# AutonomousVehicleLaboratory/vision_semantic_segmentation

Hardware: AMD Instinct MI355X
Metric: fused frames/sec/GPU (1920x1080 + 120k pts) + max|dlog-odds| vs ref (higher is better)
Workload: dtype f16 hi+lo split, MX-FP4 correction passes, fp32 accumulate

## Files before the change

### vision_semantic_segmentation_amd/csrc/experiments/seg_gemm_mx_pp.inc

```

template <int IO>
__global__ void __launch_bounds__(512) k_gemm_mx_pp(MxArgs q, int mtiles) {
    typedef f16 H;
    typedef typename Half16<H>::v8 v8;
    typedef int v8i __attribute__((ext_vector_type(8)));
    constexpr int MI = 8, BM = 256, BN = 256;
    constexpr int A_BYTES = BM * 128, W_BYTES = BN * 128;
    constexpr int W_REGION = 2 * A_BYTES, S_REGION = W_REGION + 2 * W_BYTES, S_BYTES = 4096;
    extern __shared__ __attribute__((aligned(16))) char lds[];
    const GemmArgs& p = q.g;

    const int tid = threadIdx.x, lane = tid & 63;
    const int wave = __builtin_amdgcn_readfirstlane(tid >> 6);
    const int wm = wave >> 2, wn = wave & 3;
    const int nwg = gridDim.x;
    int vb;
    {
        const int bid = blockIdx.x, xcd = bid & 7, local = bid >> 3, qq = nwg >> 3, r = nwg & 7;
        vb = (xcd < r ? xcd * (qq + 1) : r * (qq + 1) + (xcd - r) * qq) + local;
    }
    const int ntiles = p.ntiles, nmx = q.nmx;
    const int total = mtiles * ntiles;
    const int nmb = p.K / 256;
    const int nsub = 4 + nmx;
    const unsigned lds_base = lds_addr(lds);

    auto lane_now = [&]() __attribute__((always_inline)) {
        unsigned l;
        asm volatile("v_mbcnt_lo_u32_b32 %0, -1, 0\n\tv_mbcnt_hi_u32_b32 %0, -1, %0" : "=v"(l));
        return l;
    };
    int pt = vb, pmb = 0, pj = 0, issued = 0, pmbl = 0;
    long long cur_rowb16 = 0, cur_rowbq = 0, cur_asrows = 0;
    const char *cur_a16 = nullptr, *cur_aq = nullptr, *cur_as = nullptr, *cur_w16 = nullptr, *cur_wq = nullptr, *cur_ws = nullptr;
// ... 190 lines not shown
#pragma unroll
            for (int n = 0; n < 2; ++n) asm volatile("" : "+v"(acc[4 * I + m][2 * J + n]));
        __builtin_amdgcn_sched_barrier(0);
    };
    auto close = [&]() __attribute__((always_inline)) {
        asm volatile("s_barrier" ::: "memory");
        __builtin_amdgcn_sched_barrier(0);
    };
    typedef std::integral_constant<int, 0> F16;
    typedef std::integral_constant<int, 1> FP4;
    typedef std::integral_constant<int, 0> Q0;
    typedef std::integral_constant<int, 1> Q1;
    typedef std::integral_constant<int, 2> Q2;
    typedef std::integral_constant<int, 3> Q3;

    asm volatile("s_waitcnt vmcnt(0)\n\ts_barrier" ::: "memory");
    if (wm == 1) asm volatile("s_barrier" ::: "memory");
    __builtin_amdgcn_sched_barrier(0);
    for (int t = vb; t < total; t += nwg) {
        const int nt = t % ntiles, mt = t / ntiles;
        for (int mb = 0; mb < nmb; ++mb) {
            const bool last_mb = mb + 1 == nmb;
            for (int j = 0; j < 4; ++j) {
                quadrant(F16(), Q0()); close(); quadrant(F16(), Q1()); close(); quadrant(F16(), Q2()); close(); quadrant(F16(), Q3()); close();
                ++g;
            }
            for (int u = 0; u < nmx; ++u) {
                quadrant(FP4(), Q0()); close(); quadrant(FP4(), Q1()); close(); quadrant(FP4(), Q2()); close(); quadrant(FP4(), Q3());
                if (!(last_mb && u + 1 == nmx)) close();
                ++g;
            }
        }
        if (wm == 0) close();
        mx_epilogue<IO, MI>(q, acc, nt, mt, wm, wn, fr, kq);
        if (t + nwg < total) init_acc(t + nwg);
        if (wm == 1) close();
    }
    if (wm == 0) asm volatile("s_barrier" ::: "memory");
}
```

### vision_semantic_segmentation_amd/csrc/seg_gemm.hip

```cpp
#include <cstdlib>
#include <cstring>
#include <type_traits>

#include "seg_types.h"

namespace avl {
namespace {

struct GemmArgs {
    const void* A;
    const void* W;
    const float* bias;
    const void* R;
    void* C;
    int lda, ldr, ldc;
    int M, N, K;
    int relu, out_f32;
    int ntiles;
    int nsub;
    long long a_lo_delta;
    const void* R_lo;
    void* C_lo;
};

template <int NSUB> __device__ __forceinline__ bool sub_needs_a(int j) { return NSUB == 1 || j == 0 || (NSUB == 3 && j == 2); }

__device__ __forceinline__ void glds16(const void* g, void* l) {
    __builtin_amdgcn_global_load_lds((const __attribute__((address_space(1))) void*)g,
                                     (__attribute__((address_space(3))) void*)l, 16, 0, 0);
}

template <typename T, int WM, int WN>
__global__ void __launch_bounds__(WM* WN * 64) k_gemm(GemmArgs p) {
    constexpr int NW = WM * WN, BM = WM * 64, BN = WN * 64;
    constexpr int A_BYTES = BM * 128, W_BYTES = BN * 128, BUF = A_BYTES + W_BYTES;
// ... 422 lines not shown
    a.ntiles = (a.N + BN - 1) / BN;
    const int mtiles = (M + BM - 1) / BM;
    const int total = mtiles * a.ntiles;
    const int grid = total < 256 ? total : 256;
#ifdef AVL_EXPERIMENTS
    const int probe = AVL_EXP_INT("AVL_GEMM_PROBE", 0);
    if (probe >= 1 && probe <= 3 && NSUB == 1 && IO == 0) {
#define AVL_PROBE_LAUNCH(P)                                                                                                                     \
    do {                                                                                                                                        \
        (void)hipFuncSetAttribute(reinterpret_cast<const void*>(&k_gemm_ring<H, WM, WN, MI, STAGES, P>), hipFuncAttributeMaxDynamicSharedMemorySize, LDS); \
        hipLaunchKernelGGL((k_gemm_ring<H, WM, WN, MI, STAGES, P>), dim3(grid), dim3(WM * WN * 64), LDS, s, a, mtiles);                         \
    } while (0)
        if (probe == 1) AVL_PROBE_LAUNCH(1);
        else if (probe == 2) AVL_PROBE_LAUNCH(2);
        else AVL_PROBE_LAUNCH(3);
#undef AVL_PROBE_LAUNCH
    } else
#endif
        hipLaunchKernelGGL((k_gemm_ring<H, WM, WN, MI, STAGES, 0, NSUB, IO, AST>), dim3(grid), dim3(WM * WN * 64), LDS, s, a, mtiles);
    AVL_LAUNCH_CHECK();
    return AVL_OK;
}

template <typename T, int WM, int WN>
int launch_cfg(const GemmArgs& a, int mtiles, hipStream_t s) {
    constexpr int LDS = 2 * (WM * 64 + WN * 64) * 128;
    AVL_HIP_CHECK(hipFuncSetAttribute(reinterpret_cast<const void*>(&k_gemm<T, WM, WN>),
                                      hipFuncAttributeMaxDynamicSharedMemorySize, LDS));
    hipLaunchKernelGGL((k_gemm<T, WM, WN>), dim3(mtiles * a.ntiles), dim3(WM * WN * 64), LDS, s, a);
    AVL_LAUNCH_CHECK();
    return AVL_OK;
}

struct MxArgs {
    GemmArgs g;
    const char* Aq[2];
    const char* As[2];
    const char* Wq[2];
    const char* Ws[2];
    int ldaq;
    long long a_srows, w_srows;
    char* Cq[2];
    char* Cs[2];
    int ldcq;
    long long c_srows;
    int nmx;
    const char* Rq;
    const char* Rs;
    int ldrq;
    long long r_srows;
    int nmb1;
    const void* A2;
    int lda2, ldaq2;
    const char* Aq2[2];
    const char* As2[2];
    long long a_srows2;
    int stagger;
    unsigned long long* dbg;
    int same_tile;
};

__device__ __forceinline__ unsigned quantize_fp4_block(const float (&v)[16], unsigned (&q)[2]) {
    float amax = 0.f;
#pragma unroll
    for (int i = 0; i < 16; ++i) amax = fmaxf(amax, fabsf(v[i]));
    {
        const unsigned ab = __float_as_uint(amax);
        const auto r16 = __builtin_amdgcn_permlane16_swap(ab, ab, false, false);
        amax = __uint_as_float(max(r16[0], r16[1]));
    }
    const unsigned sbyte = mx_fp4_scale_byte(amax);
    const float scale = __uint_as_float(sbyte << 23);
    q[0] = q[1] = 0u;
#define AVL_FP4_PAIR(i)                                                                                  \
    q[0] = __builtin_amdgcn_cvt_scalef32_pk_fp4_f32(q[0], v[2 * (i)], v[2 * (i) + 1], scale, (i));        \
    q[1] = __builtin_amdgcn_cvt_scalef32_pk_fp4_f32(q[1], v[8 + 2 * (i)], v[8 + 2 * (i) + 1], scale, (i))
    AVL_FP4_PAIR(0); AVL_FP4_PAIR(1); AVL_FP4_PAIR(2); AVL_FP4_PAIR(3);
#undef AVL_FP4_PAIR
    return sbyte;
}

template <int IO, int MI>
__device__ __forceinline__ void mx_epilogue(const MxArgs& q, f32x4 (&acc)[MI][4], int nt, int mt, int wm, int wn, int fr, int kq) {
    typedef f16 H;
    typedef typename Half16<H>::v8 v8;
    constexpr int BM = 2 * MI * 16, BN = 256;
    const GemmArgs& p = q.g;
    const int nbase = nt * BN + wn * 64 + kq * 16;
    const bool ncol_ok = nbase + 16 <= p.N;
    const bool rsplit = p.R_lo != nullptr, csplit = p.C_lo != nullptr;
    const unsigned m0 = (unsigned)(mt * BM + wm * (MI * 16) + fr);
    const unsigned sc_r = (unsigned)(nbase >> 8) * (unsigned)q.r_srows * 8u + (unsigned)((nbase >> 5) & 7);
    const unsigned sc_c = (unsigned)(nbase >> 8) * (unsigned)q.c_srows * 8u + (unsigned)((nbase >> 5) & 7);
    v8 nr0 = {}, nr1 = {};
    uint2 npk = make_uint2(0u, 0u);
    unsigned nsb = 127u;
    auto load_res = [&](int mi) {
        const unsigned m = m0 + mi * 16;
        if (p.R && (int)m < p.M && ncol_ok) {
            const H* rp = static_cast<const H*>(p.R) + (m * (unsigned)p.ldr + (unsigned)nbase);
            nr0 = *reinterpret_cast<const v8*>(rp);
            nr1 = *reinterpret_cast<const v8*>(rp + 8);
            if (q.Rq) {
                npk = *reinterpret_cast<const uint2*>(q.Rq + (m * (unsigned)q.ldrq + (unsigned)(nbase / 2)));
                nsb = (unsigned char)q.Rs[sc_r + m * 8u];
            }
        }
    };
    load_res(0);
#pragma unroll
    for (int mi = 0; mi < MI; ++mi) {
        const unsigned m = m0 + mi * 16;
        const bool live = (int)m < p.M && ncol_ok;
        const v8 r0 = nr0, r1 = nr1;
        const uint2 pk = npk;
        const unsigned sb = nsb;
        if (mi + 1 < MI) load_res(mi + 1);
        float v[16];
#pragma unroll
        for (int nj = 0; nj < 4; ++nj)
#pragma unroll
            for (int r = 0; r < 4; ++r) v[nj * 4 + r] = acc[mi][nj][r];
        if (p.R && live) {
            float rl[16];
#pragma unroll
            for (int i = 0; i < 16; ++i) rl[i] = 0.f;
            if (rsplit) {
                const H* rlp = static_cast<const H*>(p.R_lo) + (m * (unsigned)p.ldr + (unsigned)nbase);
                const v8 l0 = *reinterpret_cast<const v8*>(rlp), l1 = *reinterpret_cast<const v8*>(rlp + 8);
#pragma unroll
                for (int i = 0; i < 8; ++i) { rl[i] = (float)l0[i]; rl[8 + i] = (float)l1[i]; }
            } else if (q.Rq) {
                typedef float v2f __attribute__((ext_vector_type(2)));
                const float sc = __uint_as_float(sb << 23);
#define AVL_FP4_DEC(w, sel, o) { const v2f d = __builtin_amdgcn_cvt_scalef32_pk_f32_fp4(w, sc, sel); rl[o] = d.x; rl[o + 1] = d.y; }
                AVL_FP4_DEC(pk.x, 0, 0) AVL_FP4_DEC(pk.x, 1, 2) AVL_FP4_DEC(pk.x, 2, 4) AVL_FP4_DEC(pk.x, 3, 6)
                AVL_FP4_DEC(pk.y, 0, 8) AVL_FP4_DEC(pk.y, 1, 10) AVL_FP4_DEC(pk.y, 2, 12) AVL_FP4_DEC(pk.y, 3, 14)
#undef AVL_FP4_DEC
            }
#pragma unroll
            for (int i = 0; i < 8; ++i) { v[i] += (float)r0[i] + rl[i]; v[8 + i] += (float)r1[i] + rl[8 + i]; }
        }
        if (p.relu) {
#pragma unroll
            for (int i = 0; i < 16; ++i) v[i] = fmaxf(v[i], 0.f);
        }
        v8 h0, h1;
#pragma unroll
        for (int i = 0; i < 8; ++i) { h0[i] = (H)v[i]; h1[i] = (H)v[8 + i]; }
        float hi[16], lo[16];
#pragma unroll
        for (int i = 0; i < 8; ++i) {
            hi[i] = (float)h0[i];
            hi[8 + i] = (float)h1[i];
            lo[i] = v[i] - hi[i];
            lo[8 + i] = v[8 + i] - hi[8 + i];
        }
        const unsigned coff = m * (unsigned)p.ldc + (unsigned)nbase;
        if (live) {
            H* cp = static_cast<H*>(p.C) + coff;
            *reinterpret_cast<v8*>(cp) = h0;
            *reinterpret_cast<v8*>(cp + 8) = h1;
        }
        if (csplit) {
            v8 l0, l1;
#pragma unroll
            for (int i = 0; i < 8; ++i) { l0[i] = (H)lo[i]; l1[i] = (H)lo[8 + i]; }
            if (live) {
                H* cl = static_cast<H*>(p.C_lo) + coff;
                *reinterpret_cast<v8*>(cl) = l0;
                *reinterpret_cast<v8*>(cl + 8) = l1;
            }
#pragma unroll
            for (int i = 0; i < 8; ++i) { lo[i] = (float)l0[i]; lo[8 + i] = (float)l1[i]; }
        }
        if constexpr (IO != 0) {
#pragma unroll
            for (int pl = 0; pl < 2; ++pl) {
                if (q.Cq[pl] == nullptr) continue;
                unsigned pq[2];
                const unsigned sq = quantize_fp4_block(pl == 0 ? hi : lo, pq);
                if (live) {
                    *reinterpret_cast<uint2*>(q.Cq[pl] + (m * (unsigned)q.ldcq + (unsigned)(nbase / 2))) = make_uint2(pq[0], pq[1]);
                    if ((kq & 1) == 0) q.Cs[pl][sc_c + m * 8u] = (char)sq;
                }
            }
        }
    }
}

template <int IO, int MI>
__global__ void __launch_bounds__(512) k_gemm_ring_mx(MxArgs q, int mtiles) {
    typedef f16 H;
    typedef typename Half16<H>::v8 v8;
    typedef int v8i __attribute__((ext_vector_type(8)));
    constexpr int WM = 2, WN = 4, STAGES = 2;
    constexpr int NW = WM * WN, BM = WM * MI * 16, BN = WN * 64;
    constexpr int A_BYTES = BM * 128, W_BYTES = BN * 128;
    constexpr int W_REGION = STAGES * A_BYTES, S_REGION = W_REGION + STAGES * W_BYTES;
    constexpr int S_BYTES = 4096;
    constexpr int A_INSTR = BM / 8 / NW, W_INSTR = BN / 8 / NW;
    extern __shared__ __attribute__((aligned(16))) char lds[];
    const GemmArgs& p = q.g;

    const int tid = threadIdx.x, lane = tid & 63;
    const int wave = __builtin_amdgcn_readfirstlane(tid >> 6);
    const int wm = wave / WN, wn = wave % WN;
    const int nwg = gridDim.x;
    int vb;
    {
        const int bid = blockIdx.x, xcd = bid & 7, local = bid >> 3, qq = nwg >> 3, r = nwg & 7;
        vb = (xcd < r ? xcd * (qq + 1) : r * (qq + 1) + (xcd - r) * qq) + local;
    }
    const int total = mtiles * p.ntiles;
    const int nmb = p.K / 256;
    const int nsub = 4 + q.nmx;
    const unsigned lds_base = lds_addr(lds);

    const int srow = lane >> 3, schunk = lane & 7;
    const unsigned ct = (unsigned)((schunk ^ srow) << 4);
    const unsigned a_lane16 = (unsigned)srow * (unsigned)(p.lda * 2) + ct, a_laneq = (unsigned)srow * (unsigned)q.ldaq + ct;
    const unsigned a_lane16_2 = (unsigned)srow * (unsigned)(q.lda2 * 2) + ct, a_laneq_2 = (unsigned)srow * (unsigned)q.ldaq2 + ct;
    unsigned w_off16[W_INSTR], w_offq[W_INSTR];
#pragma unroll
// ... 105 lines not shown
                for (int kk = 0; kk < 2; ++kk) {
                    if (kk == late && pt < total) issue();
                    int4 wf[4];
                    int ws[4];
#pragma unroll
                    for (int nj = 0; nj < 4; ++nj) {
                        wf[nj] = *reinterpret_cast<const int4*>(wbase + w_off[nj] + (((kk * 4 + kq) ^ w_key[nj]) << 4));
                        {
                            const uint2 w8 = *reinterpret_cast<const uint2*>(sbase + 2048 + (wn * 4 + (fr >> 2)) * 128 + ((fr & 3) * 4 + kq) * 8);
                            ws[nj] = (int)(((nj < 2 ? w8.x : w8.y) >> (8 * ((nj & 1) * 2 + kk))) & 0xffu);
                        }
                    }
                    const int achunk = ((kk * 4 + kq) ^ a_key) << 4;
                    int4 af = *reinterpret_cast<const int4*>(abase + achunk);
                    unsigned asw = *reinterpret_cast<const unsigned*>(sbase + a_row0 * 8 + kk * 4);
#pragma unroll
                    for (int mi = 0; mi < MI; ++mi) {
                        const int4 cur = af;
                        const int as = (int)((asw >> (8 * kq)) & 0xffu);
                        if (mi + 1 < MI) {
                            af = *reinterpret_cast<const int4*>(abase + (mi + 1) * 2048 + achunk);
                            asw = *reinterpret_cast<const unsigned*>(sbase + (a_row0 + (mi + 1) * 16) * 8 + kk * 4);
                        }
                        const v8i xa = {cur.x, cur.y, cur.z, cur.w, 0, 0, 0, 0};
#pragma unroll
                        for (int nj = 0; nj < 4; ++nj) {
                            const v8i wa = {wf[nj].x, wf[nj].y, wf[nj].z, wf[nj].w, 0, 0, 0, 0};
                            acc[mi][nj] = __builtin_amdgcn_mfma_scale_f32_16x16x128_f8f6f4(wa, xa, acc[mi][nj], 4, 4, 0, ws[nj], 0, as);
                        }
                    }
                }
            }
        }
        mx_epilogue<IO, MI>(q, acc, nt, mt, wm, wn, fr, kq);
        if (t + nwg < total) init_acc(t + nwg);
    }
}

template <int IO, int MI, int LATE, int PROBE = 0, int SPREAD = 0>
__global__ void __launch_bounds__(512) k_gemm_mx_pipe(MxArgs q, int mtiles) {
    typedef f16 H;
    typedef typename Half16<H>::v8 v8;
    typedef int v8i __attribute__((ext_vector_type(8)));
    constexpr int WM = 2, WN = 4, STAGES = 2;
    constexpr int NW = WM * WN, BM = WM * MI * 16, BN = WN * 64;
    constexpr int A_BYTES = BM * 128, W_BYTES = BN * 128;
    constexpr int W_REGION = STAGES * A_BYTES, S_REGION = W_REGION + STAGES * W_BYTES;
    constexpr int S_BYTES = 4096;
    constexpr int A_INSTR = BM / 8 / NW, W_INSTR = BN / 8 / NW;
    constexpr int NS = 2 * MI, D = 3, EV = NS - D;
    constexpr int EW = (MI == 8 && SPREAD != 5) ? 5 : EV;
    constexpr bool SPR = SPREAD == 1 || SPREAD == 2, PIN = SPREAD != 0;
    constexpr bool ONE = SPREAD == 5;
    constexpr bool MID = SPREAD == 4;
    extern __shared__ __attribute__((aligned(16))) char lds[];
    const GemmArgs& p = q.g;

    const int tid = threadIdx.x, lane = tid & 63;
    const int wave = __builtin_amdgcn_readfirstlane(tid >> 6);
    const int wm = wave / WN, wn = wave % WN;
    const int nwg = gridDim.x;
    int vb;
    {
        const int bid = blockIdx.x, xcd = bid & 7, local = bid >> 3, qq = nwg >> 3, r = nwg & 7;
        vb = (xcd < r ? xcd * (qq + 1) : r * (qq + 1) + (xcd - r) * qq) + local;
    }
    const int ntiles = p.ntiles, nmx = q.nmx;
    const int total = mtiles * ntiles;
    const int nmb = p.K / 256;
    const int nsub = 4 + nmx;
    const unsigned lds_base = lds_addr(lds);

// ... 92 lines not shown
    if (pt < total) { issue_w(); issue_a(); }
    if (pt < total) { issue_w(); issue_a(); }

    const int fr = lane & 15, kq = lane >> 4;
    const int a_row0 = wm * (MI * 16) + fr;
    const int wrow0 = wn * 64 + (fr >> 2) * 16 + (fr & 3);
    const int wkey_r = ((wrow0 >> 1) & 1) | (((wrow0 >> 4) & 3) << 1);
    const unsigned a_v0 = (unsigned)(a_row0 * 128 + ((kq ^ (a_row0 & 7)) << 4));
    const unsigned w_v0 = (unsigned)(W_REGION + wrow0 * 128 + ((kq ^ wkey_r) << 4));
    const unsigned sa_v = (unsigned)(S_REGION + a_row0 * 8 + kq);
    const unsigned sw_v = (unsigned)(S_REGION + 2048 + (wn * 4 + (fr >> 2)) * 128 + ((fr & 3) * 4 + kq) * 8);

    f32x4 acc[MI][4];
    auto init_acc = [&](int t) {
        const int nb = (t % ntiles) * BN + wn * 64 + kq * 16;
#pragma unroll
        for (int nj = 0; nj < 4; ++nj) {
            const float4 b = *reinterpret_cast<const float4*>(p.bias + nb + 4 * nj);
#pragma unroll
            for (int mi = 0; mi < MI; ++mi) acc[mi][nj] = f32x4{b.x, b.y, b.z, b.w};
        }
    };
    if (vb < total) init_acc(vb);

    int4 Af[NS], Wf[2][4];
    unsigned As[NS];
    uint2 Wsc = make_uint2(0u, 0u), Wsn = make_uint2(0u, 0u);
    auto rdA = [&](const char* slot, int kk, int mi) { return *reinterpret_cast<const int4*>(slot + (a_v0 ^ (unsigned)(kk * 64)) + mi * 2048); };
    auto rdW = [&](const char* slot, int kk, int nj) { return *reinterpret_cast<const int4*>(slot + (w_v0 ^ (unsigned)(kk * 64)) + nj * 512); };
    auto rdAs = [&](const char* slot, int kk, int mi) { return (unsigned)*reinterpret_cast<const unsigned char*>(slot + sa_v + mi * 128 + kk * 4); };
    auto rdWs = [&](const char* slot) { return *reinterpret_cast<const uint2*>(slot + sw_v); };

    int g = 0;
    unsigned long long tsum[8] = {0, 0, 0, 0, 0, 0, 0, 0}, tlast = 0;
    auto stamp = [&]() __attribute__((always_inline)) {
        unsigned long long t;
        asm volatile("s_memtime %0\n\ts_waitcnt lgkmcnt(0)" : "=s"(t)::"memory");
        return t;
    };
    bool w_sent = false;
    auto step = [&](auto kind_c, auto s_c, const bool next_q) __attribute__((always_inline)) {
        constexpr int KIND = decltype(kind_c)::value, S = decltype(s_c)::value;
        constexpr int kk = S / MI, mi = S % MI;
        const char* ab = lds + (g & 1) * A_BYTES;
        const char* wb = lds + (g & 1) * W_BYTES;
        const char* sb = lds + (g & 1) * S_BYTES;
        const char* abn = lds + ((g + 1) & 1) * A_BYTES;
        const char* wbn = lds + ((g + 1) & 1) * W_BYTES;
        const char* sbn = lds + ((g + 1) & 1) * S_BYTES;
        auto readA = [&](int t) {
            Af[t] = rdA(ab, t / MI, t % MI);
            if (KIND == 1) As[t] = rdAs(sb, t / MI, t % MI);
        };
        auto readAn = [&](int t) {
            Af[t] = rdA(abn, t / MI, t % MI);
            As[t] = rdAs(sbn, t / MI, t % MI);
        };
        if (PROBE == 3 && S == 0) { const unsigned long long t = stamp(); if (tlast) tsum[0] += t - tlast; tlast = t; tsum[5] += 1; }
        if (EW != EV && S == EW) {
            if (!SPR && !MID && LATE == 0 && !early && g > 0 && PROBE != 1 && pt < total) {
                unsigned long long t1 = 0;
                if (PROBE == 3) t1 = stamp();
                issue_a();
                if (PROBE == 3) tsum[4] += stamp() - t1;
            }
            unsigned long long t0 = 0;
            if (PROBE == 3) t0 = stamp();
// ... 100 lines not shown
            for (int nj = 0; nj < 4; ++nj) asm volatile("" : "+v"(acc[mi][nj]));
        }
        __builtin_amdgcn_sched_barrier(0);
    };
    auto substep = [&](auto kind_c, const bool next_q) __attribute__((always_inline)) {
#define AVL_STEP(N) step(kind_c, std::integral_constant<int, N>(), next_q)
        AVL_STEP(0); AVL_STEP(1); AVL_STEP(2); AVL_STEP(3); AVL_STEP(4); AVL_STEP(5); AVL_STEP(6); AVL_STEP(7);
        if constexpr (NS == 16) { AVL_STEP(8); AVL_STEP(9); AVL_STEP(10); AVL_STEP(11); AVL_STEP(12); AVL_STEP(13); AVL_STEP(14); AVL_STEP(15); }
#undef AVL_STEP
        Wsc = Wsn;
        ++g;
    };
    typedef std::integral_constant<int, 0> F16;
    typedef std::integral_constant<int, 1> FP4;

    asm volatile("s_waitcnt vmcnt(0)" ::: "memory");
    __builtin_amdgcn_s_barrier();
    for (int t = vb; t < total; t += nwg) {
        const int nt = t % ntiles, mt = t / ntiles;
        {
            const char* ab = lds + (g & 1) * A_BYTES;
            const char* wb = lds + (g & 1) * W_BYTES;
#pragma unroll
            for (int nj = 0; nj < 4; ++nj) Wf[0][nj] = rdW(wb, 0, nj);
#pragma unroll
            for (int s = 0; s < D; ++s) Af[s] = rdA(ab, 0, s);
        }
        for (int mb = 0; mb < nmb; ++mb) {
            for (int j = 0; j < 4; ++j) substep(F16(), j == 3);
            for (int u = 0; u < nmx; ++u) substep(FP4(), u + 1 < nmx);
        }
        unsigned long long te0 = 0;
        if (PROBE == 3) te0 = stamp();
        mx_epilogue<IO, MI>(q, acc, nt, mt, wm, wn, fr, kq);
        if (t + nwg < total) init_acc(t + nwg);
        if (PROBE == 3) { tsum[6] += stamp() - te0; tsum[7] += 1; tlast = 0; }
    }
    if (PROBE == 3 && q.dbg && lane == 0) {
#pragma unroll
        for (int i = 0; i < 8; ++i) q.dbg[((size_t)blockIdx.x * 8 + wave) * 8 + i] = tsum[i];
    }
}

#ifdef AVL_EXPERIMENTS
#include "experiments/seg_gemm_mx_pp.inc"
#endif

template <int IO, int MI>
int launch_ring_mx_t(const MxArgs& a0, hipStream_t s) {
    constexpr int BM = 2 * MI * 16, LDS = 2 * (BM + 256) * 128 + 2 * 4096;
    MxArgs a = a0;
    a.stagger = AVL_EXP_INT("AVL_MX_STAGGER", 1);
    a.same_tile = 0;
    a.g.ntiles = a.g.N / 256;
    const int mtiles = (a.g.M + BM - 1) / BM;
    const int total = mtiles * a.g.ntiles;
    int grid = total < 256 ? total : 256;
#ifdef AVL_EXPERIMENTS
    { const int gl = AVL_EXP_INT("AVL_MX_GRID", 0); if (gl > 0 && gl < grid) grid = gl; }
#endif
#ifdef AVL_EXPERIMENTS
    if (MI == 8) {
        const int pp = AVL_EXP_INT("AVL_MX_PP", 0);
        if (pp == 1 || (pp == 2 && a.g.K >= 1024)) {
            AVL_HIP_CHECK(hipFuncSetAttribute(reinterpret_cast<const void*>(&k_gemm_mx_pp<IO>), hipFuncAttributeMaxDynamicSharedMemorySize, LDS));
            hipLaunchKernelGGL((k_gemm_mx_pp<IO>), dim3(grid), dim3(512), LDS, s, a, mtiles);
            AVL_LAUNCH_CHECK();
            return AVL_OK;
        }
    }
#endif
    const int pipe_env = AVL_EXP_INT("AVL_MX_PIPE", -1);
    const bool pipe = pipe_env >= 0 ? pipe_env != 0 : a.g.K >= 1024;
    if (pipe) {
        constexpr int L0 = MI == 8 ? 0 : 1;
#define AVL_PIPE_LAUNCH(...)                                                                                                                   \
    do {                                                                                                                                       \
        AVL_HIP_CHECK(hipFuncSetAttribute(reinterpret_cast<const void*>(&k_gemm_mx_pipe<__VA_ARGS__>), hipFuncAttributeMaxDynamicSharedMemorySize, LDS)); \
        hipLaunchKernelGGL((k_gemm_mx_pipe<__VA_ARGS__>), dim3(grid), dim3(512), LDS, s, a, mtiles);                                           \
    } while (0)
#ifdef AVL_EXPERIMENTS
        constexpr int L1 = 2;
        const int late_env = AVL_EXP_INT("AVL_MX_LATE", -1);
        const int probe = AVL_EXP_INT("AVL_MX_PROBE", 0);
        if (MI == 8 && probe == 1) AVL_PIPE_LAUNCH(IO, 8, 0, 1);
        else if (MI == 8 && probe == 2) AVL_PIPE_LAUNCH(IO, 8, 0, 2);
        else if (MI == 8 && probe == 4) AVL_PIPE_LAUNCH(IO, 8, 0, 4);
        else if (MI == 8 && probe == 5) AVL_PIPE_LAUNCH(IO, 8, 0, 5);
        else if (MI == 8 && probe == 6) AVL_PIPE_LAUNCH(IO, 8, 0, 6);
        else if (MI == 8 && probe == 3) {
            hipStreamCaptureStatus cap = hipStreamCaptureStatusNone;
            AVL_HIP_CHECK(hipStreamIsCapturing(s, &cap));
            AVL_REQUIRE(cap == hipStreamCaptureStatusNone, "AVL_MX_PROBE=3 synchronises the stream: not while it is being captured (MODEL.HIP_GRAPH = False)");
            static unsigned long long* dbg = nullptr;
            if (!dbg) AVL_HIP_CHECK(hipHostMalloc(reinterpret_cast<void**>(&dbg), 256 * 8 * 8 * sizeof(unsigned long long), 0));
            memset(dbg, 0, 256 * 8 * 8 * sizeof(unsigned long long));
            a.dbg = dbg;
            a.same_tile = AVL_EXP_INT("AVL_MX_SAMETILE", 0);
            AVL_PIPE_LAUNCH(IO, 8, 0, 3);
            AVL_HIP_CHECK(hipStreamSynchronize(s));
            double sum[2][8] = {};
            for (int b = 0; b < grid; ++b)
                for (int w = 0; w < 8; ++w)
                    for (int i = 0; i < 8; ++i) sum[w >= 4][i] += (double)dbg[(b * 8 + w) * 8 + i];
            for (int e = 0; e < 2; ++e) {
                const double n = sum[e][5] > 0 ? sum[e][5] : 1;
                fprintf(stderr, "[mx probe] M %d N %d K %d nmx %d %s waves: cycles per sub-step %.0f | EW wait+barrier %.0f | W burst %.0f | EV wait+barrier %.0f | A burst %.0f | epilogue %.0f (x %.1f per wave)\n",
                        a.g.M, a.g.N, a.g.K, a.nmx, e ? "early (4-7)" : "late (0-3)", sum[e][0] / n, sum[e][1] / n, sum[e][2] / n, sum[e][3] / n, sum[e][4] / n,
                        sum[e][7] > 0 ? sum[e][6] / sum[e][7] : 0., sum[e][7] / (4.0 * grid));
            }
        }
        else if (late_env == L1) AVL_PIPE_LAUNCH(IO, MI, L1);
        else if (MI == 8 && AVL_EXP_INT("AVL_MX_SPREAD", 0) == 1) AVL_PIPE_LAUNCH(IO, 8, 0, 0, 1);
        else if (MI == 8 && AVL_EXP_INT("AVL_MX_SPREAD", 0) == 2) AVL_PIPE_LAUNCH(IO, 8, 0, 0, 2);
        else if (MI == 8 && AVL_EXP_INT("AVL_MX_SPREAD", 0) == 3) AVL_PIPE_LAUNCH(IO, 8, 0, 0, 3);
        else if (MI == 8 && AVL_EXP_INT("AVL_MX_SPREAD", 0) == 4) AVL_PIPE_LAUNCH(IO, 8, 0, 0, 4);
        else if (MI == 8 && AVL_EXP_INT("AVL_MX_SPREAD", 0) == 5) AVL_PIPE_LAUNCH(IO, 8, 0, 0, 5);
        else
#endif
            AVL_PIPE_LAUNCH(IO, MI, L0);
#undef AVL_PIPE_LAUNCH
    } else {
        AVL_HIP_CHECK(hipFuncSetAttribute(reinterpret_cast<const void*>(&k_gemm_ring_mx<IO, MI>), hipFuncAttributeMaxDynamicSharedMemorySize, LDS));
        hipLaunchKernelGGL((k_gemm_ring_mx<IO, MI>), dim3(grid), dim3(512), LDS, s, a, mtiles);
    }
    AVL_LAUNCH_CHECK();
    return AVL_OK;
}

int launch_ring_mx(const MxArgs& a, bool quantize_out, hipStream_t s) {
    const int force = AVL_EXP_INT("AVL_MX_TILE", 0);
    const long long t256 = (long long)((a.g.M + 255) / 256) * (a.g.N / 256);
    const bool small = force ? force == 128 : (t256 < 192 || (t256 > 256 && t256 < 384));
    if (small) return quantize_out ? launch_ring_mx_t<1, 4>(a, s) : launch_ring_mx_t<0, 4>(a, s);
    return quantize_out ? launch_ring_mx_t<1, 8>(a, s) : launch_ring_mx_t<0, 8>(a, s);
}

struct TileCfg { int bm, bn; };
inline TileCfg pick_tile(const avl_seg_op& op);
inline bool ring_eligible(const avl_seg_op& op) {
    const int M = op.out_h * op.out_w;
    return is_half(op.dtype) && op.w_layout != 1 && op.out_c > 64 && !op.out_f32 && op.out_c % 128 == 0 && op.in_rows >= (M + 255) / 256 * 256;
}
inline TileCfg pick_tile(const avl_seg_op& op) {
    if (op.out_c <= 64) return {256, 64};
    return {128, 128};
}

}

int validate_gemm(const avl_seg_op& op) {
    const int es = elem_size(op.dtype);
    AVL_REQUIRE(is_half(op.dtype) || op.dtype == AVL_F32, "GEMM dtype %d", op.dtype);
    AVL_REQUIRE(op.in && op.out && op.weight && op.bias, "GEMM has NULL buffers");
    const int M = op.out_h * op.out_w, K = op.in_c, N = op.out_c;
    AVL_REQUIRE(M > 0 && N > 0 && K > 0, "GEMM M/N/K = %d/%d/%d", M, N, K);
    AVL_REQUIRE(op.in_h * op.in_w == M, "GEMM in/out pixel counts differ (%d vs %d)", op.in_h * op.in_w, M);
    AVL_REQUIRE((K * es) % 128 == 0, "GEMM K = %d is not a multiple of %d", K, 128 / es);
    AVL_REQUIRE(op.in_ld >= K && (op.in_ld * es) % 16 == 0, "GEMM in_ld %d", op.in_ld);
    AVL_REQUIRE(op.out_ld >= N, "GEMM out_ld %d < N %d", op.out_ld, N);
    const TileCfg t = pick_tile(op);
    const int mtiles = (M + t.bm - 1) / t.bm, ntiles = (N + t.bn - 1) / t.bn;
    AVL_REQUIRE(op.in_rows >= mtiles * t.bm, "GEMM reads %d rows, input has %d allocated", mtiles * t.bm, op.in_rows);
    AVL_REQUIRE(op.w_rows >= ntiles * t.bn, "GEMM reads %d weight rows, %d allocated", ntiles * t.bn, op.w_rows);
    AVL_REQUIRE(op.out_rows >= M, "GEMM writes %d rows, output has %d", M, op.out_rows);
    if (!op.out_f32) AVL_REQUIRE((op.out_ld * es) % 16 == 0 && N % 16 == 0, "GEMM out_ld %d / N %d not 16-aligned", op.out_ld, N);
    if (op.in2) AVL_REQUIRE(op.in2_ld >= N && (op.in2_ld * es) % 16 == 0, "GEMM residual ld %d", op.in2_ld);
    if (op.out_f32) AVL_REQUIRE(!op.out_lo, "GEMM: an fp32 output has no low plane");
// ... 143 lines not shown
```

Baseline: 226.8.

## Specialize MX epilogue on residual mode and prefetch residual rows four deep

Residual handling in the MX GEMM epilogue now depends on a compile-time mode (none, hi, fp4, f16 hi+lo), chosen at launch, so runtime branches on R, R_lo and Rq are gone. Residual loads for four rows are kept in flight, with explicit vmcnt waits sized to the number of younger loads, instead of a one-row lookahead. Out-of-range rows are clamped to the last valid row rather than branched around, and the column-bound check is dropped. Trade-offs: more template instantiations, more registers held by the four-deep buffers, and the hand-counted vmcnt values are correct only if the compiler emits exactly the expected loads; a probe hook for epilogue wait time is also added.

```diff
diff --git a/vision_semantic_segmentation_amd/csrc/experiments/seg_gemm_mx_pp.inc b/vision_semantic_segmentation_amd/csrc/experiments/seg_gemm_mx_pp.inc
--- a/vision_semantic_segmentation_amd/csrc/experiments/seg_gemm_mx_pp.inc
+++ b/vision_semantic_segmentation_amd/csrc/experiments/seg_gemm_mx_pp.inc
@@ -1,5 +1,5 @@
 
-template <int IO>
+template <int EPI>
 __global__ void __launch_bounds__(512) k_gemm_mx_pp(MxArgs q, int mtiles) {
     typedef f16 H;
     typedef typename Half16<H>::v8 v8;
@@ -256,7 +256,7 @@
             }
         }
         if (wm == 0) close();
-        mx_epilogue<IO, MI>(q, acc, nt, mt, wm, wn, fr, kq);
+        mx_epilogue<EPI, MI>(q, acc, nt, mt, wm, wn, fr, kq);
         if (t + nwg < total) init_acc(t + nwg);
         if (wm == 1) close();
     }
diff --git a/vision_semantic_segmentation_amd/csrc/seg_gemm.hip b/vision_semantic_segmentation_amd/csrc/seg_gemm.hip
--- a/vision_semantic_segmentation_amd/csrc/seg_gemm.hip
+++ b/vision_semantic_segmentation_amd/csrc/seg_gemm.hip
@@ -1,6 +1,7 @@
 #include <cstdlib>
 #include <cstring>
 #include <type_traits>
+#include <utility>
 
 #include "seg_types.h"
 
@@ -489,6 +490,7 @@
     return AVL_OK;
 }
 
+constexpr int AVL_MX_STAMPS = 10;
 struct MxArgs {
     GemmArgs g;
     const char* Aq[2];
@@ -537,66 +539,92 @@
     return sbyte;
 }
 
-template <int IO, int MI>
-__device__ __forceinline__ void mx_epilogue(const MxArgs& q, f32x4 (&acc)[MI][4], int nt, int mt, int wm, int wn, int fr, int kq) {
+enum { MXR_NONE = 0, MXR_HI = 1, MXR_FP4 = 2, MXR_F16 = 3 };
+constexpr int mx_epi(int io, int res) { return io + 2 * res; }
+template <typename F, int... I>
+__device__ __forceinline__ void for_rows(F& f, std::integer_sequence<int, I...>) { (f(std::integral_constant<int, I>()), ...); }
+
+template <int EPI, int MI, int PROBE = 0>
+__device__ __forceinline__ void mx_epilogue(const MxArgs& q, f32x4 (&acc)[MI][4], int nt, int mt, int wm, int wn, int fr, int kq,
+                                            unsigned long long* tw = nullptr) {
     typedef f16 H;
     typedef typename Half16<H>::v8 v8;
+    constexpr int IO = EPI & 1, RES = EPI >> 1;
     constexpr int BM = 2 * MI * 16, BN = 256;
+    constexpr int NL = RES == MXR_NONE ? 0 : RES == MXR_HI ? 2 : 4;
+    constexpr int NS = IO ? 4 : 2;
+    constexpr int D = 4;
     const GemmArgs& p = q.g;
     const int nbase = nt * BN + wn * 64 + kq * 16;
-    const bool ncol_ok = nbase + 16 <= p.N;
-    const bool rsplit = p.R_lo != nullptr, csplit = p.C_lo != nullptr;
+    const bool csplit = p.C_lo != nullptr;
     const unsigned m0 = (unsigned)(mt * BM + wm * (MI * 16) + fr);
+    const unsigned mlast = (unsigned)(p.M - 1);
     const unsigned sc_r = (unsigned)(nbase >> 8) * (unsigned)q.r_srows * 8u + (unsigned)((nbase >> 5) & 7);
     const unsigned sc_c = (unsigned)(nbase >> 8) * (unsigned)q.c_srows * 8u + (unsigned)((nbase >> 5) & 7);
-    v8 nr0 = {}, nr1 = {};
-    uint2 npk = make_uint2(0u, 0u);
-    unsigned nsb = 127u;
-    auto load_res = [&](int mi) {
+    auto stamp = [&]() __attribute__((always_inline)) {
+        unsigned long long t;
+        asm volatile("s_memtime %0\n\ts_waitcnt lgkmcnt(0)" : "=s"(t)::"memory");
+        return t;
+    };
+    v8 rh[RES ? D : 1][2], rl[RES == MXR_F16 ? D : 1][2];
+    uint2 rq[RES == MXR_FP4 ? D : 1];
+    unsigned rs[RES == MXR_FP4 ? D : 1];
+    auto load_res = [&](int mi) __attribute__((always_inline)) {
+        const int s = mi % D;
+        const unsigned m = min(m0 + (unsigned)(mi * 16), mlast);
+        const unsigned off = m * (unsigned)p.ldr + (unsigned)nbase;
+        const H* rp = static_cast<const H*>(p.R) + off;
+        rh[s][0] = *reinterpret_cast<const v8*>(rp);
+        rh[s][1] = *reinterpret_cast<const v8*>(rp + 8);
+        if constexpr (RES == MXR_FP4) {
+            rq[s] = *reinterpret_cast<const uint2*>(q.Rq + (m * (unsigned)q.ldrq + (unsigned)(nbase / 2)));
+            rs[s] = *reinterpret_cast<const unsigned char*>(q.Rs + (sc_r + m * 8u));
+        }
+        if constexpr (RES == MXR_F16) {
+            const H* rlp = static_cast<const H*>(p.R_lo) + off;
+            rl[s][0] = *reinterpret_cast<const v8*>(rlp);
+            rl[s][1] = *reinterpret_cast<const v8*>(rlp + 8);
+        }
+    };
+    if constexpr (RES != MXR_NONE) {
+#pragma unroll
+        for (int mi = 0; mi < D; ++mi) load_res(mi);
+    }
+    auto row = [&](auto mi_c) __attribute__((always_inline)) {
+        constexpr int mi = decltype(mi_c)::value;
         const unsigned m = m0 + mi * 16;
-        if (p.R && (int)m < p.M && ncol_ok) {
-            const H* rp = static_cast<const H*>(p.R) + (m * (unsigned)p.ldr + (unsigned)nbase);
-            nr0 = *reinterpret_cast<const v8*>(rp);
-            nr1 = *reinterpret_cast<const v8*>(rp + 8);
-            if (q.Rq) {
-                npk = *reinterpret_cast<const uint2*>(q.Rq + (m * (unsigned)q.ldrq + (unsigned)(nbase / 2)));
-                nsb = (unsigned char)q.Rs[sc_r + m * 8u];
-            }
-        }
-    };
-    load_res(0);
-#pragma unroll
-    for (int mi = 0; mi < MI; ++mi) {
-        const unsigned m = m0 + mi * 16;
-        const bool live = (int)m < p.M && ncol_ok;
-        const v8 r0 = nr0, r1 = nr1;
-        const uint2 pk = npk;
-        const unsigned sb = nsb;
-        if (mi + 1 < MI) load_res(mi + 1);
+        const bool live = (int)m < p.M;
         float v[16];
 #pragma unroll
         for (int nj = 0; nj < 4; ++nj)
 #pragma unroll
             for (int r = 0; r < 4; ++r) v[nj * 4 + r] = acc[mi][nj][r];
-        if (p.R && live) {
-            float rl[16];
-#pragma unroll
-            for (int i = 0; i < 16; ++i) rl[i] = 0.f;
-            if (rsplit) {
-                const H* rlp = static_cast<const H*>(p.R_lo) + (m * (unsigned)p.ldr + (unsigned)nbase);
-                const v8 l0 = *reinterpret_cast<const v8*>(rlp), l1 = *reinterpret_cast<const v8*>(rlp + 8);
-#pragma unroll
-                for (int i = 0; i < 8; ++i) { rl[i] = (float)l0[i]; rl[8 + i] = (float)l1[i]; }
-            } else if (q.Rq) {
+        if constexpr (RES != MXR_NONE) {
+            constexpr int younger = NL * (D - 1 < MI - 1 - mi ? D - 1 : MI - 1 - mi) + NS * (mi < D ? mi : D);
+            static_assert(younger < 64, "vmcnt has 6 bits");
+            unsigned long long t0 = 0;
+            if constexpr (PROBE == 3) t0 = stamp();
+            asm volatile("s_waitcnt vmcnt(%0)" ::"n"(younger) : "memory");
+            if constexpr (PROBE == 3) { if (tw) tw[mi == 0 ? 0 : 1] += stamp() - t0; }
+            const v8 r0 = rh[mi % D][0], r1 = rh[mi % D][1];
+            float rlo[16];
+#pragma unroll
+            for (int i = 0; i < 16; ++i) rlo[i] = 0.f;
+            if constexpr (RES == MXR_F16) {
+#pragma unroll
+                for (int i = 0; i < 8; ++i) { rlo[i] = (float)rl[mi % D][0][i]; rlo[8 + i] = (float)rl[mi % D][1][i]; }
+            } else if constexpr (RES == MXR_FP4) {
                 typedef float v2f __attribute__((ext_vector_type(2)));
-                const float sc = __uint_as_float(sb << 23);
-#define AVL_FP4_DEC(w, sel, o) { const v2f d = __builtin_amdgcn_cvt_scalef32_pk_f32_fp4(w, sc, sel); rl[o] = d.x; rl[o + 1] = d.y; }
+                const uint2 pk = rq[mi % D];
+                const float sc = __uint_as_float(rs[mi % D] << 23);
+#define AVL_FP4_DEC(w, sel, o) { const v2f d = __builtin_amdgcn_cvt_scalef32_pk_f32_fp4(w, sc, sel); rlo[o] = d.x; rlo[o + 1] = d.y; }
                 AVL_FP4_DEC(pk.x, 0, 0) AVL_FP4_DEC(pk.x, 1, 2) AVL_FP4_DEC(pk.x, 2, 4) AVL_FP4_DEC(pk.x, 3, 6)
                 AVL_FP4_DEC(pk.y, 0, 8) AVL_FP4_DEC(pk.y, 1, 10) AVL_FP4_DEC(pk.y, 2, 12) AVL_FP4_DEC(pk.y, 3, 14)
 #undef AVL_FP4_DEC
             }
-#pragma unroll
-            for (int i = 0; i < 8; ++i) { v[i] += (float)r0[i] + rl[i]; v[8 + i] += (float)r1[i] + rl[8 + i]; }
+            if (mi + D < MI) load_res(mi + D);
+#pragma unroll
+            for (int i = 0; i < 8; ++i) { v[i] += (float)r0[i] + rlo[i]; v[8 + i] += (float)r1[i] + rlo[8 + i]; }
         }
         if (p.relu) {
 #pragma unroll
@@ -634,7 +662,7 @@
         if constexpr (IO != 0) {
 #pragma unroll
             for (int pl = 0; pl < 2; ++pl) {
-                if (q.Cq[pl] == nullptr) continue;
+                if (pl == 1 && q.Cq[1] == nullptr) continue;
                 unsigned pq[2];
                 const unsigned sq = quantize_fp4_block(pl == 0 ? hi : lo, pq);
                 if (live) {
@@ -643,10 +671,11 @@
                 }
             }
         }
-    }
-}
-
-template <int IO, int MI>
+    };
+    for_rows(row, std::make_integer_sequence<int, MI>());
+}
+
+template <int EPI, int MI>
 __global__ void __launch_bounds__(512) k_gemm_ring_mx(MxArgs q, int mtiles) {
     typedef f16 H;
     typedef typename Half16<H>::v8 v8;
@@ -818,12 +847,12 @@
                 }
             }
         }
-        mx_epilogue<IO, MI>(q, acc, nt, mt, wm, wn, fr, kq);
+        mx_epilogue<EPI, MI>(q, acc, nt, mt, wm, wn, fr, kq);
         if (t + nwg < total) init_acc(t + nwg);
     }
 }
 
-template <int IO, int MI, int LATE, int PROBE = 0, int SPREAD = 0>
+template <int EPI, int MI, int LATE, int PROBE = 0, int SPREAD = 0>
 __global__ void __launch_bounds__(512) k_gemm_mx_pipe(MxArgs q, int mtiles) {
     typedef f16 H;
     typedef typename Half16<H>::v8 v8;
@@ -982,7 +1011,7 @@
     auto rdWs = [&](const char* slot) { return *reinterpret_cast<const uint2*>(slot + sw_v); };
 
     int g = 0;
-    unsigned long long tsum[8] = {0, 0, 0, 0, 0, 0, 0, 0}, tlast = 0;
+    unsigned long long tsum[AVL_MX_STAMPS] = {}, tlast = 0;
     auto stamp = [&]() __attribute__((always_inline)) {
         unsigned long long t;
         asm volatile("s_memtime %0\n\ts_waitcnt lgkmcnt(0)" : "=s"(t)::"memory");
@@ -1149,13 +1178,13 @@
         }
         unsigned long long te0 = 0;
         if (PROBE == 3) te0 = stamp();
-        mx_epilogue<IO, MI>(q, acc, nt, mt, wm, wn, fr, kq);
+        mx_epilogue<EPI, MI, PROBE>(q, acc, nt, mt, wm, wn, fr, kq, tsum + 8);
         if (t + nwg < total) init_acc(t + nwg);
         if (PROBE == 3) { tsum[6] += stamp() - te0; tsum[7] += 1; tlast = 0; }
     }
     if (PROBE == 3 && q.dbg && lane == 0) {
 #pragma unroll
-        for (int i = 0; i < 8; ++i) q.dbg[((size_t)blockIdx.x * 8 + wave) * 8 + i] = tsum[i];
+        for (int i = 0; i < AVL_MX_STAMPS; ++i) q.dbg[((size_t)blockIdx.x * 8 + wave) * AVL_MX_STAMPS + i] = tsum[i];
     }
 }
 
@@ -1163,7 +1192,7 @@
 #include "experiments/seg_gemm_mx_pp.inc"
 #endif
 
-template <int IO, int MI>
+template <int EPI, int MI>
 int launch_ring_mx_t(const MxArgs& a0, hipStream_t s) {
     constexpr int BM = 2 * MI * 16, LDS = 2 * (BM + 256) * 128 + 2 * 4096;
     MxArgs a = a0;
@@ -1180,8 +1209,8 @@
     if (MI == 8) {
         const int pp = AVL_EXP_INT("AVL_MX_PP", 0);
         if (pp == 1 || (pp == 2 && a.g.K >= 1024)) {
-            AVL_HIP_CHECK(hipFuncSetAttribute(reinterpret_cast<const void*>(&k_gemm_mx_pp<IO>), hipFuncAttributeMaxDynamicSharedMemorySize, LDS));
-            hipLaunchKernelGGL((k_gemm_mx_pp<IO>), dim3(grid), dim3(512), LDS, s, a, mtiles);
+            AVL_HIP_CHECK(hipFuncSetAttribute(reinterpret_cast<const void*>(&k_gemm_mx_pp<EPI>), hipFuncAttributeMaxDynamicSharedMemorySize, LDS));
+            hipLaunchKernelGGL((k_gemm_mx_pp<EPI>), dim3(grid), dim3(512), LDS, s, a, mtiles);
             AVL_LAUNCH_CHECK();
             return AVL_OK;
         }
@@ -1200,57 +1229,71 @@
         constexpr int L1 = 2;
         const int late_env = AVL_EXP_INT("AVL_MX_LATE", -1);
         const int probe = AVL_EXP_INT("AVL_MX_PROBE", 0);
-        if (MI == 8 && probe == 1) AVL_PIPE_LAUNCH(IO, 8, 0, 1);
-        else if (MI == 8 && probe == 2) AVL_PIPE_LAUNCH(IO, 8, 0, 2);
-        else if (MI == 8 && probe == 4) AVL_PIPE_LAUNCH(IO, 8, 0, 4);
-        else if (MI == 8 && probe == 5) AVL_PIPE_LAUNCH(IO, 8, 0, 5);
-        else if (MI == 8 && probe == 6) AVL_PIPE_LAUNCH(IO, 8, 0, 6);
+        if (MI == 8 && probe == 1) AVL_PIPE_LAUNCH(EPI, 8, 0, 1);
+        else if (MI == 8 && probe == 2) AVL_PIPE_LAUNCH(EPI, 8, 0, 2);
+        else if (MI == 8 && probe == 4) AVL_PIPE_LAUNCH(EPI, 8, 0, 4);
+        else if (MI == 8 && probe == 5) AVL_PIPE_LAUNCH(EPI, 8, 0, 5);
+        else if (MI == 8 && probe == 6) AVL_PIPE_LAUNCH(EPI, 8, 0, 6);
         else if (MI == 8 && probe == 3) {
             hipStreamCaptureStatus cap = hipStreamCaptureStatusNone;
             AVL_HIP_CHECK(hipStreamIsCapturing(s, &cap));
             AVL_REQUIRE(cap == hipStreamCaptureStatusNone, "AVL_MX_PROBE=3 synchronises the stream: not while it is being captured (MODEL.HIP_GRAPH = False)");
             static unsigned long long* dbg = nullptr;
-            if (!dbg) AVL_HIP_CHECK(hipHostMalloc(reinterpret_cast<void**>(&dbg), 256 * 8 * 8 * sizeof(unsigned long long), 0));
-            memset(dbg, 0, 256 * 8 * 8 * sizeof(unsigned long long));
+            if (!dbg) AVL_HIP_CHECK(hipHostMalloc(reinterpret_cast<void**>(&dbg), 256 * 8 * AVL_MX_STAMPS * sizeof(unsigned long long), 0));
+            memset(dbg, 0, 256 * 8 * AVL_MX_STAMPS * sizeof(unsigned long long));
             a.dbg = dbg;
             a.same_tile = AVL_EXP_INT("AVL_MX_SAMETILE", 0);
-            AVL_PIPE_LAUNCH(IO, 8, 0, 3);
+            AVL_PIPE_LAUNCH(EPI, 8, 0, 3);
             AVL_HIP_CHECK(hipStreamSynchronize(s));
-            double sum[2][8] = {};
+            double sum[2][AVL_MX_STAMPS] = {};
             for (int b = 0; b < grid; ++b)
                 for (int w = 0; w < 8; ++w)
-                    for (int i = 0; i < 8; ++i) sum[w >= 4][i] += (double)dbg[(b * 8 + w) * 8 + i];
+                    for (int i = 0; i < AVL_MX_STAMPS; ++i) sum[w >= 4][i] += (double)dbg[(b * 8 + w) * AVL_MX_STAMPS + i];
             for (int e = 0; e < 2; ++e) {
                 const double n = sum[e][5] > 0 ? sum[e][5] : 1;
-                fprintf(stderr, "[mx probe] M %d N %d K %d nmx %d %s waves: cycles per sub-step %.0f | EW wait+barrier %.0f | W burst %.0f | EV wait+barrier %.0f | A burst %.0f | epilogue %.0f (x %.1f per wave)\n",
+                fprintf(stderr, "[mx probe] M %d N %d K %d nmx %d %s waves: cycles per sub-step %.0f | EW wait+barrier %.0f | W burst %.0f | EV wait+barrier %.0f | A burst %.0f | epilogue %.0f (x %.1f per wave) | epilogue entry wait %.0f | row waits %.0f | res %d\n",
                         a.g.M, a.g.N, a.g.K, a.nmx, e ? "early (4-7)" : "late (0-3)", sum[e][0] / n, sum[e][1] / n, sum[e][2] / n, sum[e][3] / n, sum[e][4] / n,
-                        sum[e][7] > 0 ? sum[e][6] / sum[e][7] : 0., sum[e][7] / (4.0 * grid));
-            }
-        }
-        else if (late_env == L1) AVL_PIPE_LAUNCH(IO, MI, L1);
-        else if (MI == 8 && AVL_EXP_INT("AVL_MX_SPREAD", 0) == 1) AVL_PIPE_LAUNCH(IO, 8, 0, 0, 1);
-        else if (MI == 8 && AVL_EXP_INT("AVL_MX_SPREAD", 0) == 2) AVL_PIPE_LAUNCH(IO, 8, 0, 0, 2);
-        else if (MI == 8 && AVL_EXP_INT("AVL_MX_SPREAD", 0) == 3) AVL_PIPE_LAUNCH(IO, 8, 0, 0, 3);
-        else if (MI == 8 && AVL_EXP_INT("AVL_MX_SPREAD", 0) == 4) AVL_PIPE_LAUNCH(IO, 8, 0, 0, 4);
-        else if (MI == 8 && AVL_EXP_INT("AVL_MX_SPREAD", 0) == 5) AVL_PIPE_LAUNCH(IO, 8, 0, 0, 5);
+                        sum[e][7] > 0 ? sum[e][6] / sum[e][7] : 0., sum[e][7] / (4.0 * grid),
+                        sum[e][7] > 0 ? sum[e][8] / sum[e][7] : 0., sum[e][7] > 0 ? sum[e][9] / sum[e][7] : 0., EPI >> 1);
+            }
+        }
+        else if (late_env == L1) AVL_PIPE_LAUNCH(EPI, MI, L1);
+        else if (MI == 8 && AVL_EXP_INT("AVL_MX_SPREAD", 0) == 1) AVL_PIPE_LAUNCH(EPI, 8, 0, 0, 1);
+        else if (MI == 8 && AVL_EXP_INT("AVL_MX_SPREAD", 0) == 2) AVL_PIPE_LAUNCH(EPI, 8, 0, 0, 2);
+        else if (MI == 8 && AVL_EXP_INT("AVL_MX_SPREAD", 0) == 3) AVL_PIPE_LAUNCH(EPI, 8, 0, 0, 3);
+        else if (MI == 8 && AVL_EXP_INT("AVL_MX_SPREAD", 0) == 4) AVL_PIPE_LAUNCH(EPI, 8, 0, 0, 4);
+        else if (MI == 8 && AVL_EXP_INT("AVL_MX_SPREAD", 0) == 5) AVL_PIPE_LAUNCH(EPI, 8, 0, 0, 5);
         else
 #endif
-            AVL_PIPE_LAUNCH(IO, MI, L0);
+            AVL_PIPE_LAUNCH(EPI, MI, L0);
 #undef AVL_PIPE_LAUNCH
     } else {
-        AVL_HIP_CHECK(hipFuncSetAttribute(reinterpret_cast<const void*>(&k_gemm_ring_mx<IO, MI>), hipFuncAttributeMaxDynamicSharedMemorySize, LDS));
-        hipLaunchKernelGGL((k_gemm_ring_mx<IO, MI>), dim3(grid), dim3(512), LDS, s, a, mtiles);
+        AVL_HIP_CHECK(hipFuncSetAttribute(reinterpret_cast<const void*>(&k_gemm_ring_mx<EPI, MI>), hipFuncAttributeMaxDynamicSharedMemorySize, LDS));
+        hipLaunchKernelGGL((k_gemm_ring_mx<EPI, MI>), dim3(grid), dim3(512), LDS, s, a, mtiles);
     }
     AVL_LAUNCH_CHECK();
     return AVL_OK;
+}
+
+template <int MI>
+int launch_ring_mx_mi(const MxArgs& a, bool quantize_out, hipStream_t s) {
+    const int res = !a.g.R ? MXR_NONE : a.Rq ? MXR_FP4 : a.g.R_lo ? MXR_F16 : MXR_HI;
+#define AVL_EPI_CASE(R) \
+    case R: return quantize_out ? launch_ring_mx_t<mx_epi(1, R), MI>(a, s) : launch_ring_mx_t<mx_epi(0, R), MI>(a, s)
+    switch (res) {
+        AVL_EPI_CASE(MXR_NONE);
+        AVL_EPI_CASE(MXR_HI);
+        AVL_EPI_CASE(MXR_FP4);
+        default: AVL_EPI_CASE(MXR_F16);
+    }
+#undef AVL_EPI_CASE
 }
 
 int launch_ring_mx(const MxArgs& a, bool quantize_out, hipStream_t s) {
     const int force = AVL_EXP_INT("AVL_MX_TILE", 0);
     const long long t256 = (long long)((a.g.M + 255) / 256) * (a.g.N / 256);
     const bool small = force ? force == 128 : (t256 < 192 || (t256 > 256 && t256 < 384));
-    if (small) return quantize_out ? launch_ring_mx_t<1, 4>(a, s) : launch_ring_mx_t<0, 4>(a, s);
-    return quantize_out ? launch_ring_mx_t<1, 8>(a, s) : launch_ring_mx_t<0, 8>(a, s);
+    return small ? launch_ring_mx_mi<4>(a, quantize_out, s) : launch_ring_mx_mi<8>(a, quantize_out, s);
 }
 
 struct TileCfg { int bm, bn; };
```

New measurement: 229.1, median of 6. Within noise of the previous version (+1.0%).
